# MrTornado24/IDE-3D

Hardware: AMD Instinct MI355X
Metric: 512x512 RGB+seg frames/s @96 depth samples (whole job) (higher is better)
Workload: dtype f32 (3x3 convs + MLPs: fp32 operands as 3 bf16 pieces, 6 products, f32 accumulate); 1 GPU; BASELINE config 2: random-init ide3d-ffhq-64-512, G.mapping + G.synthesis (64 render -> 512, 96 samples, RGB + 19-class seg) + uint8 frames, batch 4 seeds per GPU; global_batch=4, parallelism=dp1, conv_arithmetic=bf16x6, conv_arithmetic_is_library_default=True

## Files before the change

ide-3d_amd/csrc/modconv.hip:

```cpp
#include "common.h"
#include "knobs.h"
#include <stdlib.h>
#include <string.h>
#include <type_traits>

namespace ide3d {

typedef float f32x16 __attribute__((ext_vector_type(16)));

#ifdef IDE3D_MC_TRACE
__device__ unsigned long long g_mc_dbg[256];
#define IDE3D_MC_TS(k) { const unsigned long long now_ = __builtin_readcyclecounter(); mc_acc[k] += now_ - mc_last; mc_last = now_; }
#else
#define IDE3D_MC_TS(k)
#endif

enum { MODE_CONV3 = 0, MODE_CONV1 = 1, MODE_TCONV3 = 2, MODE_TCONV3A = 3, MODE_CONV3S2 = 4 };

template <int MODE> struct ModeCfg;
template <> struct ModeCfg<MODE_CONV3>  { static constexpr int KC = 4, WTAPS = 9, MAXT = 9; };
template <> struct ModeCfg<MODE_CONV1>  { static constexpr int KC = 16, WTAPS = 1, MAXT = 1; };
template <> struct ModeCfg<MODE_CONV3S2> { static constexpr int KC = 4, WTAPS = 9, MAXT = 9; };
template <> struct ModeCfg<MODE_TCONV3> { static constexpr int KC = 4, WTAPS = 9, MAXT = 4; };
template <> struct ModeCfg<MODE_TCONV3A> { static constexpr int KC = 4, WTAPS = 9, MAXT = 9; };

template <int MODE, int BIG, int TI, int PH, int PW>
struct McCfg {
    static constexpr int NWV = 4, NT = 64 * NWV;
    static constexpr int BN = TI * PH * PW;
    static_assert(BN == 64 || BN == 128 || BN == 256, "pixel tile must hold 64, 128 or 256 pixels");
    static constexpr int NCLS = (MODE == MODE_TCONV3A) ? 4 : 1;
    using MC = ModeCfg<MODE>;
    static constexpr int KC = MC::KC, WTAPS = MC::WTAPS, MAXT = MC::MAXT;
    static constexpr int WM = BIG ? 2 : 1, WN = NWV / WM;
    static constexpr int MTW = (BIG == 1) ? 2 : 1;
    static constexpr int NTW = (BN / 32) / WN;
// ... 1203 lines not shown
#pragma unroll
        for (int e = 0; e < HS_UN; ++e) xv[e] = xl[(int64_t)(c + e) * hw];
#pragma unroll
        for (int r = 0; r < HS_RB; ++r)
#pragma unroll
            for (int e = 0; e < HS_UN; ++e) acc[r] = fmaf(xv[e], wr[r][c + e], acc[r]);
    }
    for (; c < c1; ++c) {
        const float xv = xl[(int64_t)c * hw];
#pragma unroll
        for (int r = 0; r < HS_RB; ++r) acc[r] = fmaf(xv, wr[r][c], acc[r]);
    }
#pragma unroll
    for (int r = 0; r < HS_RB; ++r) s_red[ks][r][px_l] = acc[r];
    __syncthreads();
    float amax = 0.f;
    if (threadIdx.x < HS_RB * PX) {
        const int r = threadIdx.x / PX, row = row0 + r, px = (int)blockIdx.y * PX + px_l;
        float v = s_red[0][r][px_l];
#pragma unroll
        for (int q = 1; q < KS; ++q) v += s_red[q][r][px_l];
        if (row < p.cout && px < hw) {
            if (p.bias) v += p.bias[row];
            v *= p.gain;
            if (p.clamp >= 0.f) v = fminf(fmaxf(v, -p.clamp), p.clamp);
            p.y[((int64_t)n * p.cout + row) * hw + px] = v;
            amax_acc(amax, v);
        }
    }
    if (p.y_amax != nullptr) amax_raise_block(p.y_amax, n, amax, s_am);
}


constexpr int STRIP_CO = 8, STRIP_WAVES = 16;
__global__ void __launch_bounds__(256)
tconv_strip_pack_kernel(const float* __restrict__ w, int cout, int cin, int cout_pad, float* __restrict__ ws) {
    const int64_t total = (int64_t)cin * 6 * cout_pad;
    for (int64_t i = (int64_t)blockIdx.x * 256 + threadIdx.x; i < total; i += (int64_t)gridDim.x * 256) {
        const int co = (int)(i % cout_pad); const int64_t r = i / cout_pad;
        const int t = (int)(r % 6), ci = (int)(r / 6);
        const int tap = t < 3 ? 6 + t : (t - 3) * 3 + 2;
        ws[i] = co < cout ? w[((int64_t)co * cin + ci) * 9 + tap] : 0.f;
    }
}
__global__ void __launch_bounds__(256)
tconv_strip_gather_kernel(const float* __restrict__ x, int rows, int h, int w_, float* __restrict__ xs) {
    const int len = w_ + h;
    for (int64_t i = (int64_t)blockIdx.x * 256 + threadIdx.x; i < (int64_t)rows * len; i += (int64_t)gridDim.x * 256) {
        const int64_t r = i / len; const int e = (int)(i - r * len);
        xs[i] = e < w_ ? x[r * h * w_ + (int64_t)(h - 1) * w_ + e] : x[r * h * w_ + (int64_t)(e - w_) * w_ + (w_ - 1)];
    }
}
__global__ void __launch_bounds__(64 * STRIP_WAVES, 4)
tconv_strip_kernel(ide3d_modconv_params p, const float* __restrict__ ws, const float* __restrict__ xs, int cout_pad, int oh, int ow, int64_t pitch,
                   int nb_re, int nb_ro, int nb_ce) {
    __shared__ float s_red[STRIP_WAVES][STRIP_CO][64];
    __shared__ float s_am[STRIP_WAVES];
    const int h = p.h, w_ = p.w_;
    const int lane = threadIdx.x & 63, q = __builtin_amdgcn_readfirstlane((int)(threadIdx.x >> 6));
    int b = (int)blockIdx.x, kind = 0;
    if (b >= nb_re) { b -= nb_re; kind = 1; if (b >= nb_ro) { b -= nb_ro; kind = 2; if (b >= nb_ce) { b -= nb_ce; kind = 3; } } }
    const bool is_row = kind < 2, odd = kind & 1;
    const int a = b * 64 + lane;
    const int t = 2 * a + (odd ? 1 : 0);
    const bool live = t < (is_row ? ow : oh - 1);
    const int co0 = (int)blockIdx.y * STRIP_CO, n = (int)blockIdx.z;
    const int len = is_row ? w_ : h;
    const bool ok_a = live && a < len, ok_b = live && !odd && a >= 1;
    const int64_t xs_pitch = (int64_t)w_ + h;
    const float* __restrict__ xn = xs + (int64_t)n * p.cin * xs_pitch;
    const int64_t off_a = (is_row ? 0 : w_) + min(a, len - 1), off_b = (is_row ? 0 : w_) + min(max(a - 1, 0), len - 1);
    const float* __restrict__ wt = ws + (is_row ? 0 : 3) * (int64_t)cout_pad + co0;
    constexpr int STRIP_CH = 8 * STRIP_WAVES, PER_WAVE = STRIP_CH / STRIP_WAVES, WPC = 3 * STRIP_CO;
    static_assert(PER_WAVE * WPC == 3 * 64, "three weight loads per lane and chunk");
    __shared__ __attribute__((aligned(16))) float s_wt[STRIP_WAVES][PER_WAVE * WPC];
    float acc[STRIP_CO];
#pragma unroll
    for (int j = 0; j < STRIP_CO; ++j) acc[j] = 0.f;
    for (int c0 = 0; c0 < p.cin; c0 += STRIP_CH) {
        float xa[PER_WAVE], xb[PER_WAVE], scv[PER_WAVE], wreg[3];
#pragma unroll
        for (int k = 0; k < PER_WAVE; ++k) {
            const int ci = min(c0 + q + k * STRIP_WAVES, p.cin - 1);
            xa[k] = xn[(int64_t)ci * xs_pitch + off_a];
            xb[k] = odd ? 0.f : xn[(int64_t)ci * xs_pitch + off_b];
            scv[k] = p.styles ? p.styles[(int64_t)n * p.cin + ci] : 1.f;
        }
#pragma unroll
        for (int r = 0; r < 3; ++r) {
            const int e = lane + 64 * r, k = e / WPC, rem = e - k * WPC, tp = rem / STRIP_CO, jj = rem - tp * STRIP_CO;
            const int ci = c0 + q + k * STRIP_WAVES;
            wreg[r] = (ci < p.cin) ? wt[((int64_t)ci * 6 + tp) * cout_pad + jj] : 0.f;
        }
        __builtin_amdgcn_wave_barrier();
#pragma unroll
        for (int r = 0; r < 3; ++r) s_wt[q][lane + 64 * r] = wreg[r];
        __builtin_amdgcn_fence(__ATOMIC_RELEASE, "wavefront");
        __builtin_amdgcn_wave_barrier();
        __builtin_amdgcn_fence(__ATOMIC_ACQUIRE, "wavefront");
#pragma unroll
        for (int k = 0; k < PER_WAVE; ++k) {
            const float va = ok_a ? xa[k] * scv[k] : 0.f;
            const float4* wv = reinterpret_cast<const float4*>(&s_wt[q][k * WPC]);
            if (odd) {
                const float4 b0 = wv[2], b1 = wv[3];
                const float w1[STRIP_CO] = {b0.x, b0.y, b0.z, b0.w, b1.x, b1.y, b1.z, b1.w};
#pragma unroll
                for (int j = 0; j < STRIP_CO; ++j) acc[j] = fmaf(va, w1[j], acc[j]);
            } else {
                const float vb = ok_b ? xb[k] * scv[k] : 0.f;
                const float4 a0 = wv[0], a1 = wv[1], c0v = wv[4], c1v = wv[5];
                const float w0[STRIP_CO] = {a0.x, a0.y, a0.z, a0.w, a1.x, a1.y, a1.z, a1.w};
                const float w2[STRIP_CO] = {c0v.x, c0v.y, c0v.z, c0v.w, c1v.x, c1v.y, c1v.z, c1v.w};
#pragma unroll
                for (int j = 0; j < STRIP_CO; ++j) { acc[j] = fmaf(va, w0[j], acc[j]); acc[j] = fmaf(vb, w2[j], acc[j]); }
            }
        }
    }
#pragma unroll
    for (int j = 0; j < STRIP_CO; ++j) s_red[q][j][lane] = acc[j];
    __syncthreads();
    float am = 0.f;
    {
        static_assert(STRIP_CO <= STRIP_WAVES, "wave q < STRIP_CO finishes output channel co0 + q");
        float v = 0.f;
        const int qc = min(q, STRIP_CO - 1);
#pragma unroll
        for (int k = 0; k < STRIP_WAVES; ++k) v += s_red[k][qc][lane];
        const int co = co0 + q;
        if (live && q < STRIP_CO && co < p.cout) {
            v *= p.dcoefs ? p.dcoefs[(int64_t)n * p.cout + co] : 1.f;
            const int oy = is_row ? oh - 1 : t, ox = is_row ? t : ow - 1;
            p.y[((int64_t)n * p.cout + co) * ((int64_t)oh * pitch) + (int64_t)oy * pitch + ox] = v;
            amax_acc(am, v);
        }
    }
    if (p.y_amax) amax_raise_block(p.y_amax, n, am, s_am);
}

struct BlockId { int mb, tile, grp, split; };
__device__ __forceinline__ BlockId decode_block(const ConvGeom& g) {
    int bid = xcd_remap(blockIdx.x, gridDim.x);
    BlockId b;
    b.mb = bid % g.mblocks; bid /= g.mblocks;
    b.tile = bid % g.tile_base[4]; bid /= g.tile_base[4];
    b.grp = bid % g.img_groups; bid /= g.img_groups;
    b.split = bid;
    return b;
}

template <int MODE, int BIG, int TI, int PH, int PW>
__global__ void __launch_bounds__(256, (McCfg<MODE, BIG, TI, PH, PW>::NCLS * McCfg<MODE, BIG, TI, PH, PW>::MTW * McCfg<MODE, BIG, TI, PH, PW>::NTW > 8) ? 1
                                       : (TI * PH * PW <= 128 && MODE != MODE_CONV3S2) ? 3 : 2)
modconv_kernel(ide3d_modconv_params p, const float* __restrict__ wp, float* __restrict__ partial, ConvGeom g) {
    using K = McCfg<MODE, BIG, TI, PH, PW>;
    __shared__ __attribute__((aligned(16))) float s_w[2 * K::LDS_W];
    __shared__ __attribute__((aligned(16))) float s_x[2 * K::LDS_X];
    const BlockId b = decode_block(g);
    int cls = 0;
    if (MODE == MODE_TCONV3) { cls = (b.tile >= g.tile_base[1]) + (b.tile >= g.tile_base[2]) + (b.tile >= g.tile_base[3]); }
    modconv_tile<MODE, BIG, TI, PH, PW>(p, wp, partial, g, s_w, s_x, b.mb, b.tile - g.tile_base[cls], b.grp, b.split, cls, g.tiles_x[cls]);
}


#ifdef IDE3D_SP_SHARED_SIMD
constexpr bool kSpExclusive = false;
#else
constexpr bool kSpExclusive = true;
#endif
template <int MODE, int BIG, int PH, int PARTS, int WBUF, int NWV>
// ... 506 lines not shown
    if (pl.parts) {
        if (!p.weights_packed) pack_split_weights(p, pl, wp, st);
#define IDE3D_SP_DISPATCH(M) \
        do { if (pl.big == 1) { if (pl.f16) launch_split<M, 1, 2, 1>(p, pl, wp, partial, st); else if (pl.parts == 2) launch_split<M, 1, 2>(p, pl, wp, partial, st); else launch_split<M, 1, 3>(p, pl, wp, partial, st); } \
             else             { if (pl.f16) launch_split<M, 2, 2, 1>(p, pl, wp, partial, st); else if (pl.parts == 2) launch_split<M, 2, 2>(p, pl, wp, partial, st); else launch_split<M, 2, 3>(p, pl, wp, partial, st); } } while (0)
        if (pl.mode == MODE_CONV3) IDE3D_SP_DISPATCH(MODE_CONV3); else IDE3D_SP_DISPATCH(MODE_TCONV3A);
#undef IDE3D_SP_DISPATCH
    } else {
    if (!p.weights_packed) {
        hipLaunchKernelGGL(modconv_pack_kernel, dim3(stream_grid(pl.packed_floats, 256)), dim3(256), 0, st,
                           p.w, p.w_batch_stride, p.w_batch_stride ? p.n : 1, p.cout, p.cin, pl.taps, pl.bm, pl.kc, pl.mblocks, pl.cchunks, wp);
    }
#define IDE3D_MC_DISPATCH(M) \
    do { if (pl.big == 1) launch_tiles<M, 1>(p, pl, wp, partial, st); else if (pl.big == 2) launch_tiles<M, 2>(p, pl, wp, partial, st); \
         else launch_tiles<M, 0>(p, pl, wp, partial, st); } while (0)
    if (pl.mode == MODE_CONV3)       IDE3D_MC_DISPATCH(MODE_CONV3);
    else if (pl.mode == MODE_CONV1)  IDE3D_MC_DISPATCH(MODE_CONV1);
    else if (pl.mode == MODE_CONV3S2) IDE3D_MC_DISPATCH(MODE_CONV3S2);
    else if (pl.mode == MODE_TCONV3A) IDE3D_MC_DISPATCH(MODE_TCONV3A);
    else                             IDE3D_MC_DISPATCH(MODE_TCONV3);
#undef IDE3D_MC_DISPATCH
    }
    if (pl.g.split_k > 1) {
        const int64_t per = (int64_t)p.n * p.cout * pl.oh * pl.ow;
        hipLaunchKernelGGL(modconv_epilogue_kernel, dim3(stream_grid((p.y_pitch <= 0 && ((pl.oh * pl.ow) & 3) == 0) ? per / 4 : per, 256)), dim3(256), 0, st, p, partial, pl.g.split_k, pl.oh, pl.ow);
    }
    if (pl.mode == MODE_TCONV3A && !p.weights_packed) {
        hipLaunchKernelGGL(tconv_strip_pack_kernel, dim3(stream_grid(pl.strip_floats, 256)), dim3(256), 0, st, p.w, p.cout, p.cin, cdiv(p.cout, STRIP_CO) * STRIP_CO,
                           wp + pl.packed_floats + pl.strip_off);
    }
    if (pl.strip) {
        const int cout_pad = cdiv(p.cout, STRIP_CO) * STRIP_CO;
        float* const wstrip = wp + pl.packed_floats + pl.strip_off;
        const int nb_re = cdiv(p.w_ + 1, 64), nb_ro = cdiv(p.w_, 64), nb_ce = cdiv(p.h, 64), nb_co = cdiv(p.h, 64);
        float* const xs = wstrip + pl.strip_floats;
        hipLaunchKernelGGL(tconv_strip_gather_kernel, dim3(stream_grid((int64_t)p.n * p.cin * (p.h + p.w_), 256)), dim3(256), 0, st, p.x, p.n * p.cin, p.h, p.w_, xs);
        hipLaunchKernelGGL(tconv_strip_kernel, dim3(nb_re + nb_ro + nb_ce + nb_co, cout_pad / STRIP_CO, p.n), dim3(64 * STRIP_WAVES), 0, st, p, wstrip, xs, cout_pad,
                           pl.oh, pl.ow, (int64_t)(p.y_pitch > 0 ? p.y_pitch : pl.ow), nb_re, nb_ro, nb_ce);
    }
    IDE3D_CHECK_LAUNCH("modconv2d");
    return IDE3D_OK;
}

extern "C" int ide3d_modconv2d_heads(const ide3d_modconv_params* pp, const ide3d_modconv_head_epilogue* hp, void* stream) {
    using namespace ide3d;
    IDE3D_CHECK_ARG(pp != nullptr && hp != nullptr, "modconv2d_heads: null params");
    const ide3d_modconv_params& p = *pp;
    const ide3d_modconv_head_epilogue& h = *hp;
    IDE3D_CHECK_ARG(p.x && p.w && p.workspace && (p.y || h.no_activation_output) && h.w && h.y && h.workspace, "modconv2d_heads: null tensor / workspace pointer");
    int rc = check_modconv(p);
    if (rc) return rc;
    IDE3D_CHECK_ARG(p.act == 1 || p.act == 3, "modconv2d_heads: act must be linear (1) or lrelu (3)");
    IDE3D_CHECK_ARG(h.rows > 0, "modconv2d_heads: bad head rows");
    auto no_kernel = [](const char* why) { set_error("modconv2d_heads: %s", why); return IDE3D_ENOKERNEL; };
    if (knob_live("IDE3D_MODCONV_NO_HEAD_FUSION")) return no_kernel("IDE3D_MODCONV_NO_HEAD_FUSION is set");
    if (p.k != 3 || p.mode != 0 || p.w_batch_stride != 0 || p.y_amax || p.y_pitch != 0) return no_kernel("not a shared-weight 3x3 layer without side outputs");
    int arith = resolve_arith(p.arith);
    if (arith == 16 && !p.x_amax) arith = 6;
    if (arith != 6) return no_kernel("the fused form exists for bf16x6 only");
    ConvPlan pl; plan_conv(p, pl, arith);
    if (pl.parts != 3 || pl.f16 || pl.mode != MODE_CONV3 || pl.pair || pl.g.split_k != 1 || pl.g.mblocks != 1 || pl.bm != p.cout || kTiles[pl.tile].images != 1)
        return no_kernel("the layer's plan does not hold all channels of a tile in one workgroup");
    const bool tile16 = pl.big == 1 && p.cout == 128 && pl.tile == T16x16 && sp_form(pl).waves == 8;
    const bool tile32 = pl.big == 2 && p.cout == 64 && pl.tile == T32x16;
    const int ph = tile32 ? 32 : 16;
    if (!(tile16 || tile32) || p.h % ph != 0 || p.w_ % 16 != 0) return no_kernel("no fused instance for this tile");
    ide3d_modconv_params q{};
    q.x = p.y; q.w = h.w; q.bias = h.bias; q.y = h.y;
    q.n = p.n; q.cin = p.cout; q.cout = h.rows; q.h = p.h; q.w_ = p.w_; q.k = 1; q.mode = 0;
    q.act = 1; q.alpha = 0.f; q.gain = 1.f; q.clamp = h.clamp; q.w_batch_stride = (int64_t)h.rows * p.cout; q.arith = p.arith;
    const int mt = h.rows <= 32 ? 1 : 6, hcc = p.cout / 16;
// ... 86 lines not shown
```

ide-3d_amd/csrc/upfirdn2d.hip:

```cpp
#include "common.h"
#include "knobs.h"
#include <type_traits>

namespace ide3d {

template <class T>
__device__ __forceinline__ typename Elem<T>::math_t
apply_epilogue(typename Elem<T>::math_t v, const ide3d_upfirdn2d_epilogue& ep, int n, int c, int oy, int ox, int out_w) {
    using M = typename Elem<T>::math_t;
    if (ep.add) v += Elem<T>::ld((const T*)ep.add + n * ep.add_stride[0] + c * ep.add_stride[1] + oy * ep.add_stride[2] + ox * ep.add_stride[3]);
    if (ep.noise) v += (M)(ep.noise[oy * out_w + ox] * ep.noise_strength);
    if (ep.fused_act) {
        if (ep.bias) v += Elem<T>::ld((const T*)ep.bias + c);
        if (ep.act == 3) v = (v > 0) ? v : v * (M)ep.alpha;
        v *= (M)ep.act_gain;
        if (ep.clamp >= 0.f) v = (v > (M)ep.clamp) ? (M)ep.clamp : ((v < -(M)ep.clamp) ? -(M)ep.clamp : v);
    }
    return v;
}

template <class T, int NO>
__device__ __forceinline__ void epilogue_row(typename Elem<T>::math_t (&row)[NO], const ide3d_upfirdn2d_epilogue& ep,
                                             const T* add_plane, typename Elem<T>::math_t bias, int oy, int ox0, int out_w, bool full) {
    using M = typename Elem<T>::math_t;
// ... 311 lines not shown
#pragma unroll
                        for (int tx_ = 0; tx_ < AX::ntaps(rx); ++tx_) {
                            const int wy = (UY > 1) ? cy + AY::off(ry) + ty_ : cy * DY + ty_;
                            const int wx = (UX > 1) ? cx + AX::off(rx) + tx_ : cx * DX + tx_;
                            acc += win[wy][wx] * g[AY::first(ry) + ty_ * UY][AX::first(rx) + tx_ * UX];
                        }
                    row[cx * UX + rx] = acc;
                }
            const int qx = qx0 + tx * CX;
            const int ox0 = (UX > 1) ? qx * UX + p.pad_x0 : qx;
            T* yr = yp + oy * p.y_stride[2];
            constexpr int NO = CX * UX;
            const bool full = ox0 >= 0 && ox0 + NO <= p.out_w;
            epilogue_row<T, NO>(row, ep, add_plane, bias, oy, ox0, p.out_w, full);
#pragma unroll
            for (int j = 0; j < NO; ++j)
                if (full || (ox0 + j >= 0 && ox0 + j < p.out_w)) amax_t = fmaxf(amax_t, fabsf((float)row[j]));
            if constexpr (sizeof(T) == 4 && NO == 4) {
                if (full && ((reinterpret_cast<uintptr_t>(yr + ox0) & 15) == 0)) {
                    float4 v4 = make_float4(row[0], row[1], row[2], row[3]);
                    *reinterpret_cast<float4*>(yr + ox0) = v4;
                    continue;
                }
            }
#pragma unroll
            for (int j = 0; j < NO; ++j) {
                const int ox = ox0 + j;
                if (ox >= 0 && ox < p.out_w) Elem<T>::st(yr + ox, row[j]);
            }
        }
    if (ep.y_amax) amax_raise_block(ep.y_amax, n, amax_t, reinterpret_cast<float*>(s_in));
}

__global__ void __launch_bounds__(256)
fir44_kernel(ide3d_upfirdn2d_params p, ide3d_upfirdn2d_epilogue ep, int tiles_x, int tiles_y) {
    constexpr int TCX = 128, TCY = 32, LW = 136, LH = TCY + 3, NV = LW / 4, NLD = (LH * NV + 255) / 256;
    __shared__ __attribute__((aligned(16))) float s_in[LH * LW];
    float g[4][4];
#pragma unroll
    for (int ky = 0; ky < 4; ++ky)
#pragma unroll
        for (int kx = 0; kx < 4; ++kx) {
            const int fy = p.flip ? ky : 3 - ky, fx = p.flip ? kx : 3 - kx;
            g[ky][kx] = p.f[fy * p.f_stride[0] + fx * p.f_stride[1]] * p.gain;
        }
    int bid = xcd_remap(blockIdx.x, gridDim.x);
    const int tx_i = bid % tiles_x; bid /= tiles_x;
    const int ty_i = bid % tiles_y; bid /= tiles_y;
    const int n = bid / p.c, c = bid % p.c;
    const int in_x0 = tx_i * TCX - p.pad_x0, in_y0 = ty_i * TCY - p.pad_y0;
    const int x_al = in_x0 & ~3, xoff = in_x0 - x_al;
    const float* __restrict__ xp = (const float*)p.x + n * p.x_stride[0] + c * p.x_stride[1];
    const unsigned pitch = (unsigned)p.x_stride[2];
    const int w4 = (p.in_w + 3) & ~3;
    {
        float4 v4[NLD];
        int gy[NLD], gx[NLD];
#pragma unroll
        for (int k = 0; k < NLD; ++k) {
            const int idx = (int)threadIdx.x + k * 256;
            const int ly = idx / NV, lv = idx - ly * NV;
            gy[k] = in_y0 + ly; gx[k] = x_al + 4 * lv;
            const unsigned cy_ = (unsigned)min(max(gy[k], 0), p.in_h - 1), cx_ = (unsigned)min(max(gx[k], 0), w4 - 4);
            v4[k] = *reinterpret_cast<const float4*>(xp + (cy_ * pitch + cx_));
        }
#pragma unroll
        for (int k = 0; k < NLD; ++k) {
            const int idx = (int)threadIdx.x + k * 256;
            if (idx < LH * NV) {
                const bool rowok = (unsigned)gy[k] < (unsigned)p.in_h;
                float4 w = v4[k];
                w.x = (rowok && (unsigned)(gx[k] + 0) < (unsigned)p.in_w) ? w.x : 0.f;
                w.y = (rowok && (unsigned)(gx[k] + 1) < (unsigned)p.in_w) ? w.y : 0.f;
                w.z = (rowok && (unsigned)(gx[k] + 2) < (unsigned)p.in_w) ? w.z : 0.f;
                w.w = (rowok && (unsigned)(gx[k] + 3) < (unsigned)p.in_w) ? w.w : 0.f;
                *reinterpret_cast<float4*>(s_in + 4 * idx) = w;
            }
        }
    }
    __syncthreads();
    const int tx = threadIdx.x & 31, ty = threadIdx.x >> 5;
    float win[7][7];
    {
        const float* wsrc = s_in + (ty * 4) * LW + tx * 4 + xoff;
#pragma unroll
        for (int wy = 0; wy < 7; ++wy)
#pragma unroll
            for (int wx = 0; wx < 7; ++wx) win[wy][wx] = wsrc[wy * LW + wx];
    }
    const bool has_noise = ep.noise != nullptr, act_on = ep.fused_act != 0;
    const float nstr = ep.noise_strength;
    const float bias = (act_on && ep.bias) ? ((const float*)ep.bias)[c] : 0.f;
    const bool lrelu = act_on && ep.act == 3, lrelu_max = lrelu && ep.alpha >= 0.f && ep.alpha <= 1.f;
    const float alpha = ep.alpha, again = act_on ? ep.act_gain : 1.f;
    const bool clamp_on = act_on && ep.clamp >= 0.f;
    const float cl = ep.clamp;
    float* __restrict__ yp = (float*)p.y + n * p.y_stride[0] + c * p.y_stride[1];
    const unsigned ypitch = (unsigned)p.y_stride[2];
    const int ox0 = tx_i * TCX + tx * 4, oy0 = ty_i * TCY + ty * 4;
    const bool full = ox0 + 4 <= p.out_w;
    float amax_t = 0.f;
    if (full) {
#pragma unroll
        for (int cy = 0; cy < 4; ++cy) {
            const int oy = oy0 + cy;
            if (oy >= p.out_h) break;
            float row[4];
#pragma unroll
            for (int cx = 0; cx < 4; ++cx) {
                float acc = 0.f;
#pragma unroll
                for (int ky = 0; ky < 4; ++ky)
#pragma unroll
                    for (int kx = 0; kx < 4; ++kx) acc += win[cy + ky][cx + kx] * g[ky][kx];
                row[cx] = acc;
            }
            if (has_noise) {
                const float4 a = *reinterpret_cast<const float4*>(ep.noise + ((unsigned)oy * (unsigned)p.out_w + (unsigned)ox0));
                row[0] += a.x * nstr; row[1] += a.y * nstr; row[2] += a.z * nstr; row[3] += a.w * nstr;
            }
            if (act_on) {
#pragma unroll
                for (int j = 0; j < 4; ++j) {
                    float v = row[j] + bias;
                    if (lrelu_max) v = fmaxf(v, v * alpha);
                    else if (lrelu) v = (v > 0.f) ? v : v * alpha;
                    v *= again;
                    if (clamp_on) v = (v > cl) ? cl : ((v < -cl) ? -cl : v);
                    row[j] = v;
                }
            }
#pragma unroll
            for (int j = 0; j < 4; ++j) amax_t = fmaxf(amax_t, fabsf(row[j]));
            *reinterpret_cast<float4*>(yp + ((unsigned)oy * ypitch + (unsigned)ox0)) = make_float4(row[0], row[1], row[2], row[3]);
        }
    }
    if (ep.y_amax) amax_raise_block(ep.y_amax, n, amax_t, s_in);
}

static bool fir44_applies(const ide3d_upfirdn2d_params& p, const ide3d_upfirdn2d_epilogue& ep) {
    const bool off = knob_live("IDE3D_FIR_NO_LEAN");
    if (off || p.dtype != IDE3D_F32 || p.f_w != 4 || p.f_h != 4 || p.up_x != 1 || p.up_y != 1 || p.down_x != 1 || p.down_y != 1) return false;
    if (p.x_stride[3] != 1 || p.y_stride[3] != 1 || ep.add || p.out_w <= 64 || (p.out_w & 3)) return false;
    const int64_t pitch = p.x_stride[2], w4 = (p.in_w + 3) & ~3;
    if ((pitch & 3) || pitch < w4 || w4 > (p.in_w > p.x_row_floats ? p.in_w : p.x_row_floats)) return false;
    if ((reinterpret_cast<uintptr_t>(p.x) & 15) || (p.x_stride[0] & 3) || (p.x_stride[1] & 3)) return false;
    if ((reinterpret_cast<uintptr_t>(p.y) & 15) || (p.y_stride[0] & 3) || (p.y_stride[1] & 3) || (p.y_stride[2] & 3)) return false;
    if (ep.noise && (reinterpret_cast<uintptr_t>(ep.noise) & 15)) return false;
    if (pitch * p.in_h >= (1ll << 29) || p.y_stride[2] * (int64_t)p.out_h >= (1ll << 29) || (int64_t)p.out_w * p.out_h >= (1ll << 29)) return false;
    if (p.x_stride[2] <= 0 || p.y_stride[2] <= 0) return false;
    return true;
}

static int launch_fir44(const ide3d_upfirdn2d_params& p, const ide3d_upfirdn2d_epilogue& ep, hipStream_t st) {
    const int tiles_x = cdiv(p.out_w, 128), tiles_y = cdiv(p.out_h, 32);
    const int64_t nblocks = (int64_t)tiles_x * tiles_y * p.n * p.c;
    if (nblocks > 0x7fffffff) { set_error("upfirdn2d: grid too large"); return IDE3D_EINVAL; }
    hipLaunchKernelGGL(fir44_kernel, dim3((unsigned)nblocks), dim3(256), 0, st, p, ep, tiles_x, tiles_y);
    IDE3D_CHECK_LAUNCH("upfirdn2d (fir44)");
    return IDE3D_OK;
}

__global__ void __launch_bounds__(256)
fir_up2_kernel(ide3d_upfirdn2d_params p, ide3d_upfirdn2d_epilogue ep, int tiles_x, int tiles_y) {
    using AX = Axis<2, 1, 4>;
    constexpr int TCX = 64, TCY = 16, LW = 72, LH = TCY + 2, NV = LW / 4, NLD = (LH * NV + 255) / 256;
    static_assert(AX::window(TCX) + 3 <= LW && AX::NT == 2 && AX::window(2) == 4, "window of the 4-tap polyphase filter");
    __shared__ __attribute__((aligned(16))) float s_in[LH * LW];
    float g[4][4];
#pragma unroll
    for (int ky = 0; ky < 4; ++ky)
#pragma unroll
        for (int kx = 0; kx < 4; ++kx) {
            const int fy = p.flip ? ky : 3 - ky, fx = p.flip ? kx : 3 - kx;
            g[ky][kx] = p.f[fy * p.f_stride[0] + fx * p.f_stride[1]] * p.gain;
        }
    int bid = xcd_remap(blockIdx.x, gridDim.x);
    const int tx_i = bid % tiles_x; bid /= tiles_x;
    const int ty_i = bid % tiles_y; bid /= tiles_y;
    const int n = bid / p.c, c = bid % p.c;
    const int qx0 = floordiv(-p.pad_x0, 2) + tx_i * TCX, qy0 = floordiv(-p.pad_y0, 2) + ty_i * TCY;
    const int x_al = qx0 & ~3, xoff = qx0 - x_al;
    const float* __restrict__ xp = (const float*)p.x + n * p.x_stride[0] + c * p.x_stride[1];
    const unsigned pitch = (unsigned)p.x_stride[2];
    const int w4 = (p.in_w + 3) & ~3;
    {
        float4 v4[NLD];
        int gy[NLD], gx[NLD];
#pragma unroll
        for (int k = 0; k < NLD; ++k) {
            const int idx = (int)threadIdx.x + k * 256;
// ... 1 lines not shown
            gy[k] = qy0 + ly; gx[k] = x_al + 4 * lv;
            const unsigned cy_ = (unsigned)min(max(gy[k], 0), p.in_h - 1), cx_ = (unsigned)min(max(gx[k], 0), w4 - 4);
            v4[k] = *reinterpret_cast<const float4*>(xp + (cy_ * pitch + cx_));
        }
#pragma unroll
        for (int k = 0; k < NLD; ++k) {
            const int idx = (int)threadIdx.x + k * 256;
            if (idx < LH * NV) {
                const bool rowok = (unsigned)gy[k] < (unsigned)p.in_h;
                float4 w = v4[k];
                w.x = (rowok && (unsigned)(gx[k] + 0) < (unsigned)p.in_w) ? w.x : 0.f;
                w.y = (rowok && (unsigned)(gx[k] + 1) < (unsigned)p.in_w) ? w.y : 0.f;
                w.z = (rowok && (unsigned)(gx[k] + 2) < (unsigned)p.in_w) ? w.z : 0.f;
                w.w = (rowok && (unsigned)(gx[k] + 3) < (unsigned)p.in_w) ? w.w : 0.f;
                *reinterpret_cast<float4*>(s_in + 4 * idx) = w;
            }
        }
    }
    __syncthreads();
    const int tx = threadIdx.x & 31, ty = threadIdx.x >> 5;
    float win[4][4];
    {
        const float* wsrc = s_in + (ty * 2) * LW + tx * 2 + xoff;
#pragma unroll
        for (int wy = 0; wy < 4; ++wy)
#pragma unroll
            for (int wx = 0; wx < 4; ++wx) win[wy][wx] = wsrc[wy * LW + wx];
    }
    const bool has_add = ep.add != nullptr, has_noise = ep.noise != nullptr, act_on = ep.fused_act != 0;
    const float nstr = ep.noise_strength;
    const float bias = (act_on && ep.bias) ? ((const float*)ep.bias)[c] : 0.f;
    const bool lrelu = act_on && ep.act == 3, lrelu_max = lrelu && ep.alpha >= 0.f && ep.alpha <= 1.f;
    const float alpha = ep.alpha, again = act_on ? ep.act_gain : 1.f;
    const bool clamp_on = act_on && ep.clamp >= 0.f;
    const float cl = ep.clamp;
    float* __restrict__ yp = (float*)p.y + n * p.y_stride[0] + c * p.y_stride[1];
    const float* __restrict__ ap = has_add ? (const float*)ep.add + n * ep.add_stride[0] + c * ep.add_stride[1] : nullptr;
    const unsigned ypitch = (unsigned)p.y_stride[2], apitch = (unsigned)ep.add_stride[2];
    const int ox0 = (qx0 + tx * 2) * 2 + p.pad_x0;
    const bool full = ox0 >= 0 && ox0 + 4 <= p.out_w;
    float amax_t = 0.f;
    if (full) {
#pragma unroll
        for (int cy = 0; cy < 2; ++cy)
#pragma unroll
            for (int ry = 0; ry < 2; ++ry) {
                const int oy = (qy0 + ty * 2 + cy) * 2 + ry + p.pad_y0;
                if (oy < 0 || oy >= p.out_h) continue;
                float row[4];
#pragma unroll
                for (int cx = 0; cx < 2; ++cx)
#pragma unroll
                    for (int rx = 0; rx < 2; ++rx) {
                        float acc = 0.f;
#pragma unroll
                        for (int ty_ = 0; ty_ < 2; ++ty_)
#pragma unroll
                            for (int tx_ = 0; tx_ < 2; ++tx_)
                                acc += win[cy + AX::off(ry) + ty_][cx + AX::off(rx) + tx_] * g[AX::first(ry) + ty_ * 2][AX::first(rx) + tx_ * 2];
                        row[cx * 2 + rx] = acc;
                    }
                if (has_add) {
                    const float4 a = *reinterpret_cast<const float4*>(ap + ((unsigned)oy * apitch + (unsigned)ox0));
                    row[0] += a.x; row[1] += a.y; row[2] += a.z; row[3] += a.w;
                }
                if (has_noise) {
                    const float4 a = *reinterpret_cast<const float4*>(ep.noise + ((unsigned)oy * (unsigned)p.out_w + (unsigned)ox0));
                    row[0] += a.x * nstr; row[1] += a.y * nstr; row[2] += a.z * nstr; row[3] += a.w * nstr;
                }
                if (act_on) {
#pragma unroll
                    for (int j = 0; j < 4; ++j) {
                        float v = row[j] + bias;
                        if (lrelu_max) v = fmaxf(v, v * alpha);
                        else if (lrelu) v = (v > 0.f) ? v : v * alpha;
                        v *= again;
                        if (clamp_on) v = (v > cl) ? cl : ((v < -cl) ? -cl : v);
                        row[j] = v;
                    }
                }
#pragma unroll
                for (int j = 0; j < 4; ++j) amax_t = fmaxf(amax_t, fabsf(row[j]));
                *reinterpret_cast<float4*>(yp + ((unsigned)oy * ypitch + (unsigned)ox0)) = make_float4(row[0], row[1], row[2], row[3]);
            }
    }
    if (ep.y_amax) amax_raise_block(ep.y_amax, n, amax_t, s_in);
}

static bool fir_up2_applies(const ide3d_upfirdn2d_params& p, const ide3d_upfirdn2d_epilogue& ep) {
    const bool off = knob_live("IDE3D_FIR_NO_LEAN");
    if (off || p.dtype != IDE3D_F32 || p.f_w != 4 || p.f_h != 4 || p.up_x != 2 || p.up_y != 2 || p.down_x != 1 || p.down_y != 1) return false;
    if (p.x_stride[3] != 1 || p.y_stride[3] != 1 || (p.out_w & 3) || (p.in_w & 3)) return false;
    if (p.pad_x0 & 1) return false;
    const int64_t pitch = p.x_stride[2];
    if ((pitch & 3) || pitch < p.in_w || pitch <= 0 || p.y_stride[2] <= 0) return false;
    if ((reinterpret_cast<uintptr_t>(p.x) & 15) || (p.x_stride[0] & 3) || (p.x_stride[1] & 3)) return false;
    if ((reinterpret_cast<uintptr_t>(p.y) & 15) || (p.y_stride[0] & 3) || (p.y_stride[1] & 3) || (p.y_stride[2] & 3)) return false;
    if (ep.add && (ep.add_stride[3] != 1 || (reinterpret_cast<uintptr_t>(ep.add) & 15) || (ep.add_stride[0] & 3) || (ep.add_stride[1] & 3) || (ep.add_stride[2] & 3) ||
                   ep.add_stride[2] <= 0 || ep.add_stride[2] * (int64_t)p.out_h >= (1ll << 29))) return false;
    if (ep.noise && (reinterpret_cast<uintptr_t>(ep.noise) & 15)) return false;
    if (pitch * p.in_h >= (1ll << 29) || p.y_stride[2] * (int64_t)p.out_h >= (1ll << 29) || (int64_t)p.out_w * p.out_h >= (1ll << 29)) return false;
    return true;
}

static int launch_fir_up2(const ide3d_upfirdn2d_params& p, const ide3d_upfirdn2d_epilogue& ep, hipStream_t st) {
    auto cells = [](int out, int pad0) { return floordiv(out - 1 - pad0, 2) - floordiv(-pad0, 2) + 1; };
    const int tiles_x = cdiv(cells(p.out_w, p.pad_x0), 64), tiles_y = cdiv(cells(p.out_h, p.pad_y0), 16);
    const int64_t nblocks = (int64_t)tiles_x * tiles_y * p.n * p.c;
    if (nblocks > 0x7fffffff) { set_error("upfirdn2d: grid too large"); return IDE3D_EINVAL; }
    hipLaunchKernelGGL(fir_up2_kernel, dim3((unsigned)nblocks), dim3(256), 0, st, p, ep, tiles_x, tiles_y);
    IDE3D_CHECK_LAUNCH("upfirdn2d (fir_up2)");
    return IDE3D_OK;
}

template <class T, int UX, int UY, int DX, int DY, int FW, int FH, int CX, int CY>
// ... 116 lines not shown
```

Measured before the change: 952.1 frames/s.

## Restructure tconv strip kernel and specialize fir44 epilogue with direct-to-LDS loads

The transposed-conv border strip kernel now folds the batch into the block index and computes even and odd outputs in one pass. Styles are pre-multiplied during the gather, and the wave count and channel chunking adapt to cin, with LDS allocated dynamically. The fir44 upsample kernel gains global_load_lds fills for interior tiles and template specializations for the common lrelu/clamp epilogue that skip the amax work. Amax accumulation is also gated in the up2 path. Together these cut launch and grid fragmentation and per-element branching, at the cost of more template variants and per-image amax reduction through shared atomics.

```diff
diff --git a/ide-3d_amd/csrc/modconv.hip b/ide-3d_amd/csrc/modconv.hip
--- a/ide-3d_amd/csrc/modconv.hip
+++ b/ide-3d_amd/csrc/modconv.hip
@@ -2,6 +2,7 @@
 #include "knobs.h"
 #include <stdlib.h>
 #include <string.h>
+#include <algorithm>
 #include <type_traits>
 
 namespace ide3d {
@@ -1271,7 +1272,7 @@
 }
 
 
-constexpr int STRIP_CO = 8, STRIP_WAVES = 16;
+constexpr int STRIP_CO = 8, STRIP_MAX_WAVES = 16;
 __global__ void __launch_bounds__(256)
 tconv_strip_pack_kernel(const float* __restrict__ w, int cout, int cin, int cout_pad, float* __restrict__ ws) {
     const int64_t total = (int64_t)cin * 6 * cout_pad;
@@ -1283,98 +1284,112 @@
     }
 }
 __global__ void __launch_bounds__(256)
-tconv_strip_gather_kernel(const float* __restrict__ x, int rows, int h, int w_, float* __restrict__ xs) {
+tconv_strip_gather_kernel(const float* __restrict__ x, const float* __restrict__ styles, int rows, int h, int w_, float* __restrict__ xs) {
     const int len = w_ + h;
     for (int64_t i = (int64_t)blockIdx.x * 256 + threadIdx.x; i < (int64_t)rows * len; i += (int64_t)gridDim.x * 256) {
         const int64_t r = i / len; const int e = (int)(i - r * len);
-        xs[i] = e < w_ ? x[r * h * w_ + (int64_t)(h - 1) * w_ + e] : x[r * h * w_ + (int64_t)(e - w_) * w_ + (w_ - 1)];
-    }
-}
-__global__ void __launch_bounds__(64 * STRIP_WAVES, 4)
-tconv_strip_kernel(ide3d_modconv_params p, const float* __restrict__ ws, const float* __restrict__ xs, int cout_pad, int oh, int ow, int64_t pitch,
-                   int nb_re, int nb_ro, int nb_ce) {
-    __shared__ float s_red[STRIP_WAVES][STRIP_CO][64];
-    __shared__ float s_am[STRIP_WAVES];
+        const float v = e < w_ ? x[r * h * w_ + (int64_t)(h - 1) * w_ + e] : x[r * h * w_ + (int64_t)(e - w_) * w_ + (w_ - 1)];
+        xs[i] = styles ? v * styles[r] : v;
+    }
+}
+template <int NCH>
+__global__ void __launch_bounds__(64 * STRIP_MAX_WAVES, 4)
+tconv_strip_kernel(ide3d_modconv_params p, const float* __restrict__ ws, const float* __restrict__ xs, int cout_pad, int oh, int ow, int64_t pitch, int nb_row) {
+    extern __shared__ __attribute__((aligned(16))) float s_strip[];
+    constexpr int WPC = 3 * STRIP_CO, CHW = 8 * WPC;
+    static_assert(CHW == 3 * 64 && STRIP_CO == 8, "three weight loads per lane and chunk");
     const int h = p.h, w_ = p.w_;
-    const int lane = threadIdx.x & 63, q = __builtin_amdgcn_readfirstlane((int)(threadIdx.x >> 6));
-    int b = (int)blockIdx.x, kind = 0;
-    if (b >= nb_re) { b -= nb_re; kind = 1; if (b >= nb_ro) { b -= nb_ro; kind = 2; if (b >= nb_ce) { b -= nb_ce; kind = 3; } } }
-    const bool is_row = kind < 2, odd = kind & 1;
-    const int a = b * 64 + lane;
-    const int t = 2 * a + (odd ? 1 : 0);
-    const bool live = t < (is_row ? ow : oh - 1);
-    const int co0 = (int)blockIdx.y * STRIP_CO, n = (int)blockIdx.z;
-    const int len = is_row ? w_ : h;
-    const bool ok_a = live && a < len, ok_b = live && !odd && a >= 1;
-    const int64_t xs_pitch = (int64_t)w_ + h;
-    const float* __restrict__ xn = xs + (int64_t)n * p.cin * xs_pitch;
-    const int64_t off_a = (is_row ? 0 : w_) + min(a, len - 1), off_b = (is_row ? 0 : w_) + min(max(a - 1, 0), len - 1);
+    const int lane = threadIdx.x & 63, q = __builtin_amdgcn_readfirstlane((int)(threadIdx.x >> 6)), nwaves = (int)(blockDim.x >> 6);
+    const bool is_row = (int)blockIdx.x < nb_row;
+    const int b = is_row ? (int)blockIdx.x : (int)blockIdx.x - nb_row;
+    const int per = is_row ? w_ + 1 : h, len = is_row ? w_ : h;
+    const int i = b * 64 + lane;
+    const bool live = i < p.n * per;
+    const int n = min(i / per, p.n - 1), a = i - (i / per) * per;
+    const bool ok_a = live && a < len, ok_b = live && a >= 1;
+    const int co0 = (int)blockIdx.y * STRIP_CO;
+    const int xs_pitch = w_ + h;
+    const float* __restrict__ xl = xs + (int64_t)n * p.cin * xs_pitch + (is_row ? 0 : w_);
+    const int off_a = min(a, len - 1), off_b = min(max(a - 1, 0), len - 1);
     const float* __restrict__ wt = ws + (is_row ? 0 : 3) * (int64_t)cout_pad + co0;
-    constexpr int STRIP_CH = 8 * STRIP_WAVES, PER_WAVE = STRIP_CH / STRIP_WAVES, WPC = 3 * STRIP_CO;
-    static_assert(PER_WAVE * WPC == 3 * 64, "three weight loads per lane and chunk");
-    __shared__ __attribute__((aligned(16))) float s_wt[STRIP_WAVES][PER_WAVE * WPC];
-    float acc[STRIP_CO];
-#pragma unroll
-    for (int j = 0; j < STRIP_CO; ++j) acc[j] = 0.f;
-    for (int c0 = 0; c0 < p.cin; c0 += STRIP_CH) {
-        float xa[PER_WAVE], xb[PER_WAVE], scv[PER_WAVE], wreg[3];
-#pragma unroll
-        for (int k = 0; k < PER_WAVE; ++k) {
-            const int ci = min(c0 + q + k * STRIP_WAVES, p.cin - 1);
-            xa[k] = xn[(int64_t)ci * xs_pitch + off_a];
-            xb[k] = odd ? 0.f : xn[(int64_t)ci * xs_pitch + off_b];
-            scv[k] = p.styles ? p.styles[(int64_t)n * p.cin + ci] : 1.f;
-        }
-#pragma unroll
-        for (int r = 0; r < 3; ++r) {
-            const int e = lane + 64 * r, k = e / WPC, rem = e - k * WPC, tp = rem / STRIP_CO, jj = rem - tp * STRIP_CO;
-            const int ci = c0 + q + k * STRIP_WAVES;
-            wreg[r] = (ci < p.cin) ? wt[((int64_t)ci * 6 + tp) * cout_pad + jj] : 0.f;
+    float* const s_w = s_strip + q * (NCH * CHW);
+    float ae[STRIP_CO], ao[STRIP_CO];
+#pragma unroll
+    for (int j = 0; j < STRIP_CO; ++j) { ae[j] = 0.f; ao[j] = 0.f; }
+    for (int c0 = q * (8 * NCH); c0 < p.cin; c0 += nwaves * (8 * NCH)) {
+        float xa[NCH][8], xb[NCH][8], wreg[NCH][3];
+#pragma unroll
+        for (int ch = 0; ch < NCH; ++ch) {
+#pragma unroll
+            for (int k = 0; k < 8; ++k) {
+                const int64_t ci = min(c0 + ch * 8 + k, p.cin - 1);
+                xa[ch][k] = xl[ci * xs_pitch + off_a];
+                xb[ch][k] = xl[ci * xs_pitch + off_b];
+            }
+#pragma unroll
+            for (int r = 0; r < 3; ++r) {
+                const int e = lane + 64 * r, k = e / WPC, rem = e - k * WPC, tp = rem / STRIP_CO, jj = rem - tp * STRIP_CO;
+                const int64_t ci = min(c0 + ch * 8 + k, p.cin - 1);
+                wreg[ch][r] = wt[(ci * 6 + tp) * cout_pad + jj];
+            }
         }
         __builtin_amdgcn_wave_barrier();
 #pragma unroll
-        for (int r = 0; r < 3; ++r) s_wt[q][lane + 64 * r] = wreg[r];
-        __builtin_amdgcn_fence(__ATOMIC_RELEASE, "wavefront");
-        __builtin_amdgcn_wave_barrier();
-        __builtin_amdgcn_fence(__ATOMIC_ACQUIRE, "wavefront");
-#pragma unroll
-        for (int k = 0; k < PER_WAVE; ++k) {
-            const float va = ok_a ? xa[k] * scv[k] : 0.f;
-            const float4* wv = reinterpret_cast<const float4*>(&s_wt[q][k * WPC]);
-            if (odd) {
-                const float4 b0 = wv[2], b1 = wv[3];
-                const float w1[STRIP_CO] = {b0.x, b0.y, b0.z, b0.w, b1.x, b1.y, b1.z, b1.w};
-#pragma unroll
-                for (int j = 0; j < STRIP_CO; ++j) acc[j] = fmaf(va, w1[j], acc[j]);
-            } else {
-                const float vb = ok_b ? xb[k] * scv[k] : 0.f;
-                const float4 a0 = wv[0], a1 = wv[1], c0v = wv[4], c1v = wv[5];
-                const float w0[STRIP_CO] = {a0.x, a0.y, a0.z, a0.w, a1.x, a1.y, a1.z, a1.w};
-                const float w2[STRIP_CO] = {c0v.x, c0v.y, c0v.z, c0v.w, c1v.x, c1v.y, c1v.z, c1v.w};
-#pragma unroll
-                for (int j = 0; j < STRIP_CO; ++j) { acc[j] = fmaf(va, w0[j], acc[j]); acc[j] = fmaf(vb, w2[j], acc[j]); }
-            }
-        }
-    }
-#pragma unroll
-    for (int j = 0; j < STRIP_CO; ++j) s_red[q][j][lane] = acc[j];
+        for (int ch = 0; ch < NCH; ++ch) {
+#pragma unroll
+            for (int r = 0; r < 3; ++r) s_w[ch * CHW + lane + 64 * r] = wreg[ch][r];
+            __builtin_amdgcn_fence(__ATOMIC_RELEASE, "wavefront");
+            __builtin_amdgcn_wave_barrier();
+            __builtin_amdgcn_fence(__ATOMIC_ACQUIRE, "wavefront");
+#pragma unroll
+            for (int k = 0; k < 8; ++k) {
+                if (c0 + ch * 8 + k < p.cin) {
+                    const float va = ok_a ? xa[ch][k] : 0.f, vb = ok_b ? xb[ch][k] : 0.f;
+                    const float4* wv = reinterpret_cast<const float4*>(s_w + ch * CHW + k * WPC);
+                    const float4 a0 = wv[0], a1 = wv[1], b0 = wv[2], b1 = wv[3], d0 = wv[4], d1 = wv[5];
+                    const float w0[STRIP_CO] = {a0.x, a0.y, a0.z, a0.w, a1.x, a1.y, a1.z, a1.w};
+                    const float w1[STRIP_CO] = {b0.x, b0.y, b0.z, b0.w, b1.x, b1.y, b1.z, b1.w};
+                    const float w2[STRIP_CO] = {d0.x, d0.y, d0.z, d0.w, d1.x, d1.y, d1.z, d1.w};
+#pragma unroll
+                    for (int j = 0; j < STRIP_CO; ++j) {
+                        ae[j] = fmaf(va, w0[j], ae[j]);
+                        ae[j] = fmaf(vb, w2[j], ae[j]);
+                        ao[j] = fmaf(va, w1[j], ao[j]);
+                    }
+                }
+            }
+        }
+    }
+    __syncthreads();
+#pragma unroll
+    for (int j = 0; j < STRIP_CO; ++j) {
+        s_strip[(q * 2 * STRIP_CO + 2 * j) * 64 + lane] = ae[j];
+        s_strip[(q * 2 * STRIP_CO + 2 * j + 1) * 64 + lane] = ao[j];
+    }
     __syncthreads();
     float am = 0.f;
-    {
-        static_assert(STRIP_CO <= STRIP_WAVES, "wave q < STRIP_CO finishes output channel co0 + q");
+    for (int r = q; r < 2 * STRIP_CO; r += nwaves) {
         float v = 0.f;
-        const int qc = min(q, STRIP_CO - 1);
-#pragma unroll
-        for (int k = 0; k < STRIP_WAVES; ++k) v += s_red[k][qc][lane];
-        const int co = co0 + q;
-        if (live && q < STRIP_CO && co < p.cout) {
+        for (int k = 0; k < nwaves; ++k) v += s_strip[(k * 2 * STRIP_CO + r) * 64 + lane];
+        const int co = co0 + (r >> 1), t = 2 * a + (r & 1);
+        if (live && co < p.cout && t < (is_row ? ow : oh - 1)) {
             v *= p.dcoefs ? p.dcoefs[(int64_t)n * p.cout + co] : 1.f;
             const int oy = is_row ? oh - 1 : t, ox = is_row ? t : ow - 1;
             p.y[((int64_t)n * p.cout + co) * ((int64_t)oh * pitch) + (int64_t)oy * pitch + ox] = v;
             amax_acc(am, v);
         }
     }
-    if (p.y_amax) amax_raise_block(p.y_amax, n, am, s_am);
+    if (p.y_amax) {
+        unsigned* const s_am = reinterpret_cast<unsigned*>(s_strip);
+        const int n_first = (b * 64) / per;
+        __syncthreads();
+        if (threadIdx.x < 64) s_am[threadIdx.x] = 0u;
+        __syncthreads();
+        if (am > 0.f) atomicMax(&s_am[n - n_first], __float_as_uint(am));
+        __syncthreads();
+        if (threadIdx.x < 64 && n_first + (int)threadIdx.x < p.n && s_am[threadIdx.x] != 0u)
+            amax_raise(p.y_amax, n_first + (int)threadIdx.x, __uint_as_float(s_am[threadIdx.x]));
+    }
 }
 
 struct BlockId { int mb, tile, grp, split; };
@@ -1947,11 +1962,17 @@
     if (pl.strip) {
         const int cout_pad = cdiv(p.cout, STRIP_CO) * STRIP_CO;
         float* const wstrip = wp + pl.packed_floats + pl.strip_off;
-        const int nb_re = cdiv(p.w_ + 1, 64), nb_ro = cdiv(p.w_, 64), nb_ce = cdiv(p.h, 64), nb_co = cdiv(p.h, 64);
+        const int nb_row = (int)cdiv64((int64_t)p.n * (p.w_ + 1), 64), nb_col = (int)cdiv64((int64_t)p.n * p.h, 64);
+        int nch = 2;
+        while (nch > 1 && (int64_t)(nb_row + nb_col) * (cout_pad / STRIP_CO) * std::min(STRIP_MAX_WAVES, cdiv(p.cin, 8 * nch)) < 2 * 4 * kNumCU) nch /= 2;
+        const int waves = std::min(STRIP_MAX_WAVES, cdiv(p.cin, 8 * nch));
+        const size_t lds = (size_t)waves * 2 * STRIP_CO * 64 * sizeof(float);
+        const dim3 grid(nb_row + nb_col, cout_pad / STRIP_CO), block(64 * waves);
+        const int64_t ypitch = p.y_pitch > 0 ? p.y_pitch : pl.ow;
         float* const xs = wstrip + pl.strip_floats;
-        hipLaunchKernelGGL(tconv_strip_gather_kernel, dim3(stream_grid((int64_t)p.n * p.cin * (p.h + p.w_), 256)), dim3(256), 0, st, p.x, p.n * p.cin, p.h, p.w_, xs);
-        hipLaunchKernelGGL(tconv_strip_kernel, dim3(nb_re + nb_ro + nb_ce + nb_co, cout_pad / STRIP_CO, p.n), dim3(64 * STRIP_WAVES), 0, st, p, wstrip, xs, cout_pad,
-                           pl.oh, pl.ow, (int64_t)(p.y_pitch > 0 ? p.y_pitch : pl.ow), nb_re, nb_ro, nb_ce);
+        hipLaunchKernelGGL(tconv_strip_gather_kernel, dim3(stream_grid((int64_t)p.n * p.cin * (p.h + p.w_), 256)), dim3(256), 0, st, p.x, p.styles, p.n * p.cin, p.h, p.w_, xs);
+        if (nch == 2)      hipLaunchKernelGGL(tconv_strip_kernel<2>, grid, block, lds, st, p, wstrip, xs, cout_pad, pl.oh, pl.ow, ypitch, nb_row);
+        else               hipLaunchKernelGGL(tconv_strip_kernel<1>, grid, block, lds, st, p, wstrip, xs, cout_pad, pl.oh, pl.ow, ypitch, nb_row);
     }
     IDE3D_CHECK_LAUNCH("modconv2d");
     return IDE3D_OK;
diff --git a/ide-3d_amd/csrc/upfirdn2d.hip b/ide-3d_amd/csrc/upfirdn2d.hip
--- a/ide-3d_amd/csrc/upfirdn2d.hip
+++ b/ide-3d_amd/csrc/upfirdn2d.hip
@@ -367,10 +367,12 @@
     if (ep.y_amax) amax_raise_block(ep.y_amax, n, amax_t, reinterpret_cast<float*>(s_in));
 }
 
+template <int FORM>
 __global__ void __launch_bounds__(256)
 fir44_kernel(ide3d_upfirdn2d_params p, ide3d_upfirdn2d_epilogue ep, int tiles_x, int tiles_y) {
     constexpr int TCX = 128, TCY = 32, LW = 136, LH = TCY + 3, NV = LW / 4, NLD = (LH * NV + 255) / 256;
-    __shared__ __attribute__((aligned(16))) float s_in[LH * LW];
+    constexpr int DMA_UNITS = (LH * NV + 63) / 64 * 64;
+    __shared__ __attribute__((aligned(16))) float s_in[DMA_UNITS * 4];
     float g[4][4];
 #pragma unroll
     for (int ky = 0; ky < 4; ++ky)
@@ -388,7 +390,20 @@
     const float* __restrict__ xp = (const float*)p.x + n * p.x_stride[0] + c * p.x_stride[1];
     const unsigned pitch = (unsigned)p.x_stride[2];
     const int w4 = (p.in_w + 3) & ~3;
-    {
+    if (in_y0 >= 0 && in_y0 + LH <= p.in_h && x_al >= 0 && x_al + LW <= p.in_w) {
+        const int wid = __builtin_amdgcn_readfirstlane((int)(threadIdx.x >> 6));
+#pragma unroll
+        for (int k = 0; k < NLD; ++k) {
+            const int idx0 = wid * 64 + k * 256;
+            if (idx0 < LH * NV) {
+                const int idx = min(idx0 + (int)(threadIdx.x & 63), LH * NV - 1);
+                const int ly = idx / NV, lv = idx - ly * NV;
+                __builtin_amdgcn_global_load_lds((const __attribute__((address_space(1))) void*)(xp + ((unsigned)(in_y0 + ly) * pitch + (unsigned)(x_al + 4 * lv))),
+                                                 (__attribute__((address_space(3))) void*)(s_in + 4 * idx0), 16, 0, 0);
+            }
+        }
+        asm volatile("s_waitcnt vmcnt(0)" ::: "memory");
+    } else {
         float4 v4[NLD];
         int gy[NLD], gx[NLD];
 #pragma unroll
@@ -423,12 +438,12 @@
 #pragma unroll
             for (int wx = 0; wx < 7; ++wx) win[wy][wx] = wsrc[wy * LW + wx];
     }
-    const bool has_noise = ep.noise != nullptr, act_on = ep.fused_act != 0;
+    const bool has_noise = ep.noise != nullptr, act_on = FORM ? true : ep.fused_act != 0;
     const float nstr = ep.noise_strength;
     const float bias = (act_on && ep.bias) ? ((const float*)ep.bias)[c] : 0.f;
-    const bool lrelu = act_on && ep.act == 3, lrelu_max = lrelu && ep.alpha >= 0.f && ep.alpha <= 1.f;
+    const bool lrelu = act_on && (FORM ? true : ep.act == 3), lrelu_max = lrelu && (FORM ? true : ep.alpha >= 0.f && ep.alpha <= 1.f);
     const float alpha = ep.alpha, again = act_on ? ep.act_gain : 1.f;
-    const bool clamp_on = act_on && ep.clamp >= 0.f;
+    const bool clamp_on = FORM ? FORM == 2 : act_on && ep.clamp >= 0.f, want_amax = FORM ? false : ep.y_amax != nullptr;
     const float cl = ep.clamp;
     float* __restrict__ yp = (float*)p.y + n * p.y_stride[0] + c * p.y_stride[1];
     const unsigned ypitch = (unsigned)p.y_stride[2];
@@ -465,12 +480,11 @@
                     row[j] = v;
                 }
             }
-#pragma unroll
-            for (int j = 0; j < 4; ++j) amax_t = fmaxf(amax_t, fabsf(row[j]));
+            if (want_amax) amax_t = fmaxf(fmaxf(fmaxf(amax_t, fabsf(row[0])), fabsf(row[1])), fmaxf(fabsf(row[2]), fabsf(row[3])));
             *reinterpret_cast<float4*>(yp + ((unsigned)oy * ypitch + (unsigned)ox0)) = make_float4(row[0], row[1], row[2], row[3]);
         }
     }
-    if (ep.y_amax) amax_raise_block(ep.y_amax, n, amax_t, s_in);
+    if (want_amax) amax_raise_block(ep.y_amax, n, amax_t, s_in);
 }
 
 static bool fir44_applies(const ide3d_upfirdn2d_params& p, const ide3d_upfirdn2d_epilogue& ep) {
@@ -491,7 +505,10 @@
     const int tiles_x = cdiv(p.out_w, 128), tiles_y = cdiv(p.out_h, 32);
     const int64_t nblocks = (int64_t)tiles_x * tiles_y * p.n * p.c;
     if (nblocks > 0x7fffffff) { set_error("upfirdn2d: grid too large"); return IDE3D_EINVAL; }
-    hipLaunchKernelGGL(fir44_kernel, dim3((unsigned)nblocks), dim3(256), 0, st, p, ep, tiles_x, tiles_y);
+    const bool layer_form = ep.fused_act && ep.act == 3 && ep.alpha >= 0.f && ep.alpha <= 1.f && !ep.y_amax;
+    if (layer_form && ep.clamp >= 0.f) hipLaunchKernelGGL(fir44_kernel<2>, dim3((unsigned)nblocks), dim3(256), 0, st, p, ep, tiles_x, tiles_y);
+    else if (layer_form)               hipLaunchKernelGGL(fir44_kernel<1>, dim3((unsigned)nblocks), dim3(256), 0, st, p, ep, tiles_x, tiles_y);
+    else                               hipLaunchKernelGGL(fir44_kernel<0>, dim3((unsigned)nblocks), dim3(256), 0, st, p, ep, tiles_x, tiles_y);
     IDE3D_CHECK_LAUNCH("upfirdn2d (fir44)");
     return IDE3D_OK;
 }
@@ -559,7 +576,7 @@
     const float bias = (act_on && ep.bias) ? ((const float*)ep.bias)[c] : 0.f;
     const bool lrelu = act_on && ep.act == 3, lrelu_max = lrelu && ep.alpha >= 0.f && ep.alpha <= 1.f;
     const float alpha = ep.alpha, again = act_on ? ep.act_gain : 1.f;
-    const bool clamp_on = act_on && ep.clamp >= 0.f;
+    const bool clamp_on = act_on && ep.clamp >= 0.f, want_amax = ep.y_amax != nullptr;
     const float cl = ep.clamp;
     float* __restrict__ yp = (float*)p.y + n * p.y_stride[0] + c * p.y_stride[1];
     const float* __restrict__ ap = has_add ? (const float*)ep.add + n * ep.add_stride[0] + c * ep.add_stride[1] : nullptr;
@@ -606,8 +623,7 @@
                         row[j] = v;
                     }
                 }
-#pragma unroll
-                for (int j = 0; j < 4; ++j) amax_t = fmaxf(amax_t, fabsf(row[j]));
+                if (want_amax) amax_t = fmaxf(fmaxf(fmaxf(amax_t, fabsf(row[0])), fabsf(row[1])), fmaxf(fabsf(row[2]), fabsf(row[3])));
                 *reinterpret_cast<float4*>(yp + ((unsigned)oy * ypitch + (unsigned)ox0)) = make_float4(row[0], row[1], row[2], row[3]);
             }
     }
```

Measured after the change: 956.1 frames/s (median of 6 runs). Within noise of the previous version (+0.4%).
